# johncai117/Meta-Fine-Tuning

Hardware: AMD Instinct MI355X
Metric: episodes/sec at 5-way N-shot (ResNet10+GNN) per GPU and 1/2/4/8-GPU node (higher is better)
Workload: dtype f32

## Files before the change

### meta-fine-tuning_amd/csrc/conv_igemm.hip

```cpp
#include "mft_common.h"
#include "mft_hip_testing.h"

int mft_stem_conv_dispatch(const float* in, const float* w, float* out, int n_img, int H, int W, int w_ld,
                           hipStream_t s);
int mft_skinny_fwd_dispatch(const float* in, int ldi, const float* w, float* out, int ldo, int n_img, int H, int W,
                            int Cin, int Cout, int KH, int KW, int stride, int pad, int imgs_per_group,
                            long long w_group_stride, hipStream_t s);
void mft_skinny_set_dgrad_slices(int n);
void mft_skinny_set_tap(int v);
void mft_skinny_set_x3(int v);
void mft_skinny_set_nw(int v);
void mft_bn_small_set_rows(int rows);
void mft_bn_fwd_small_set_rows(int rows);
void mft_skinny_set_lines(int v);
int mft_skinny_dgrad_dispatch(const float* dy, int ldy, const float* w, float* dx, int ldx, int n_img, int H, int W,
                              int Cin, int Cout, int KH, int KW, int stride, int pad, int imgs_per_group,
                              long long w_group_stride, hipStream_t s);

namespace {

struct ConvArgs {
    const float* in;
    const float* w;
    const float* bias;
    float* out;
    int ldi, ldo;
    int H, W, Cin, OH, OW, Cout, KH, KW, stride, pad;
    int Kpad;
    int Ktot;
    int rows_per_group;
    int imgs_per_group;
    int tiles_n;
    long long wgs;
    int bt_stride;
    int ksplit;
    float* ws;
    int parity;
};

constexpr int BK = 32;
constexpr int LDS_LD = 36;
int g_dgrad_parity = 1;
int g_wgrad_tile = 64;
int g_conv_tile = 0;
int g_wgrad_pol = 7;
int g_wgrad_trim = 1;
int g_wgrad_rows = 1;
int g_wgrad_early = 1;
int g_wgrad_min_lds_kb = 0;
int g_skinny = 1;
int g_stem_fast = 1;

template <int BM, int BN, int WM, int WN, bool STEM, bool BT>
__global__ __launch_bounds__(256) void conv_igemm_kernel(ConvArgs p) {
    constexpr int TM = BM / WM / 32;
    constexpr int TN = BN / WN / 32;
    constexpr int PA = BM / 32;
    constexpr int PB = BN / 32;
    extern __shared__ __attribute__((aligned(16))) float smem[];

    const int tid = threadIdx.x;
    const int lane = tid & 63;
    const int wave = tid >> 6;
    const int wm = wave / WN, wn = wave % WN;
    const int r = lane & 31, h = lane >> 5;

    int tile_id = blockIdx.x;
    if (gridDim.y == 1) {
        const int nwg = gridDim.x, q = nwg >> 3, rmd = nwg & 7;
        const int xcd = tile_id & 7, slot = tile_id >> 3;
        tile_id = xcd * q + (xcd < rmd ? xcd : rmd) + slot;
    }
    const int nt = tile_id % p.tiles_n;
    const int mt = tile_id / p.tiles_n;
    const bool par = BT && p.parity != 0;
    const int g = par ? 0 : blockIdx.y;
    const int ph = par ? (int)(blockIdx.y >> 1) : 0, pw = par ? (int)(blockIdx.y & 1) : 0;
    const int Hc = par ? (p.OH - ph + 1) / 2 : p.OH, Wc = par ? (p.OW - pw + 1) / 2 : p.OW;
    const int rows = par ? p.imgs_per_group * Hc * Wc : p.rows_per_group;
    const int m0 = mt * BM, n0 = nt * BN;
    if (par && m0 >= rows) return;
    const int kh0 = par ? ((ph - p.pad) & 1) : 0, kw0 = par ? ((pw - p.pad) & 1) : 0;
    const int nkh = par ? (p.KH - kh0 + 1) / 2 : p.KH, nkw = par ? (p.KW - kw0 + 1) / 2 : p.KW;

    const int lrow = tid >> 3;
    const int c4 = (tid & 7) * 4;
    const int ohw = Hc * Wc;

    long long a_base[PA];
    int a_ih0[PA], a_iw0[PA];
    bool a_ok[PA];
// ... 1043 lines not shown
    a.Ktot = KH * KW * Cin;
    a.Kpad = (a.Ktot + 31) / 32 * 32;
    a.imgs_per_group = imgs_per_group;
    a.rows_per_group = imgs_per_group * a.OH * a.OW;
    a.wgs = (groups > 1) ? w_group_stride : 0;
    a.tiles_n = 0;
    a.bt_stride = 1;
    a.ksplit = 1; a.ws = nullptr; a.parity = 0;
    if (ws != nullptr && !stem && ldo % 4 == 0) {
        a.ksplit = conv_ksplit(a.rows_per_group, Cout, a.Kpad, groups);
        a.ws = ws;
    }
    hipStream_t s = (hipStream_t)stream;
    if (stem) {
        if (g_stem_fast && KH == 7 && KW == 7 && stride == 2 && pad == 3 && Cout == 64 && ldi == 3 && ldo == 64 &&
            bias == nullptr && (W == 84 || W == 224)) {
            const int rc = mft_stem_conv_dispatch(in, w, out, n_img, H, W, a.Kpad, s);
            if (rc != MFT_EINVAL) return rc;
        }
        return launch_conv<128, 64, 2, 2, true>(a, groups, s);
    }
    if (g_skinny && groups > 1 && w_group_stride != 0 && bias == nullptr && ws == nullptr) {
        const int rc = mft_skinny_fwd_dispatch(in, ldi, w, out, ldo, n_img, H, W, Cin, Cout, KH, KW, stride, pad,
                                               imgs_per_group, w_group_stride, s);
        if (rc != MFT_EINVAL) return rc;
    }
    int tile = g_conv_tile;
    if (tile == 0) tile = (Cout >= 64) ? 4 : 5;
    switch (tile) {
        case 1: return launch_conv<128, 128, 2, 2, false>(a, groups, s);
        case 2: return launch_conv<128, 64, 2, 2, false>(a, groups, s);
        case 3: return launch_conv<64, 128, 2, 2, false>(a, groups, s);
        case 4: return launch_conv<64, 64, 2, 2, false>(a, groups, s);
        default: return launch_conv<128, 32, 4, 1, false>(a, groups, s);
    }
}

extern "C" int mft_conv2d_nhwc(const float* in, int ldi, const float* w, const float* bias, float* out, int ldo,
                               int n_img, int H, int W, int Cin, int Cout, int KH, int KW, int stride, int pad,
                               int imgs_per_group, long long w_group_stride, void* stream) {
    return conv2d_impl(in, ldi, w, bias, out, ldo, n_img, H, W, Cin, Cout, KH, KW, stride, pad, imgs_per_group, w_group_stride,
                       nullptr, stream);
}

extern "C" long long mft_conv_ksplit_ws_floats(long long rows, int cols, int K) {
    const int s = conv_ksplit(rows, cols, K);
    return s > 1 ? (long long)s * rows * cols : 0;
}

extern "C" long long mft_conv_ksplit_grouped_ws_floats(long long rows_per_group, int cols, int K, int groups) {
    const int s = conv_ksplit(rows_per_group, cols, K, groups);
    return s > 1 ? (long long)s * groups * rows_per_group * cols : 0;
}

extern "C" int mft_conv2d_nhwc_ksplit_grouped(const float* in, int ldi, const float* w, float* out, int ldo, int n_img, int H, int W,
                                              int Cin, int Cout, int KH, int KW, int stride, int pad, int imgs_per_group,
                                              long long w_group_stride, float* ws, void* stream) {
    if (ws == nullptr || imgs_per_group <= 0) return MFT_EINVAL;
    return conv2d_impl(in, ldi, w, nullptr, out, ldo, n_img, H, W, Cin, Cout, KH, KW, stride, pad, imgs_per_group, w_group_stride, ws,
                       stream);
}

extern "C" int mft_conv2d_nhwc_ksplit(const float* in, int ldi, const float* w, const float* bias, float* out, int ldo,
                                      int n_img, int H, int W, int Cin, int Cout, int KH, int KW, int stride, int pad, float* ws,
                                      void* stream) {
    return conv2d_impl(in, ldi, w, bias, out, ldo, n_img, H, W, Cin, Cout, KH, KW, stride, pad, 0, 0, ws, stream);
}

extern "C" int mft_has_experiments(void) {
#ifdef MFT_EXPERIMENTS
    return 1;
#else
    return 0;
#endif
}

extern "C" int mft_debug_set_conv_tile(int tile) {
#ifndef MFT_EXPERIMENTS
    if (tile == 9502 || tile == 9504 || tile == 9505) return MFT_EINVAL;
    if (tile >= 9000 && tile < 9100 && tile != 9003 && tile != 9007) return MFT_EINVAL;
    if (tile > 4000 && tile < 5000) return MFT_EINVAL;
#endif
    if (tile >= 11000) { mft_bn_small_set_rows(tile - 11000); mft_bn_fwd_small_set_rows(tile - 11000); }
    else if (tile >= 9800) g_dgrad_parity = tile - 9800;
    else if (tile >= 9700) mft_skinny_set_lines(tile - 9700);
    else if (tile >= 9600) g_wgrad_trim = tile - 9600;
    else if (tile >= 9500) g_wgrad_rows = tile - 9500;
    else if (tile >= 9100) mft_skinny_set_nw(tile - 9100);
    else if (tile >= 9000) g_wgrad_pol = tile - 9000;
    else if (tile >= 8000) mft_skinny_set_x3(tile - 8000);
    else if (tile >= 7000) mft_skinny_set_tap(tile - 7000);
    else if (tile >= 6000) mft_skinny_set_dgrad_slices(tile - 6000);
    else if (tile >= 5000) g_wgrad_early = tile - 5000;
    else if (tile >= 4000) g_wgrad_min_lds_kb = tile - 4000;
    else if (tile >= 3000) g_skinny = tile - 3000;
    else if (tile >= 2100) g_stem_wgrad_strips = tile - 2100;
    else if (tile >= 2000) g_stem_fast = tile - 2000;
    else if (tile >= 1000) g_wgrad_tile = tile - 1000;
    else g_conv_tile = tile;
    return 0;
}

extern "C" int mft_debug_set_x3_tile(int t);

extern "C" void mft_wgrad_fwd_set_exact(int on);
extern "C" int mft_debug_reset(void) {
    mft_wgrad_fwd_set_exact(0);
    mft_wgrad_fwd_set_xcd(1);
    g_dgrad_parity = 1; g_wgrad_trim = 1; g_wgrad_rows = 1; g_wgrad_tile = 64; g_conv_tile = 0; g_wgrad_pol = 7; g_wgrad_early = 1; g_wgrad_min_lds_kb = 0; g_skinny = 1; g_stem_fast = 1; g_stem_wgrad_strips = 1;
    mft_skinny_set_lines(1); mft_skinny_set_nw(0); mft_skinny_set_x3(1); mft_skinny_set_tap(1); mft_skinny_set_dgrad_slices(1);
    mft_debug_set_x3_tile(0); mft_debug_set_x3_tile(10); mft_debug_set_x3_tile(21); mft_debug_set_x3_tile(31); mft_debug_set_x3_tile(41);
    mft_bn_small_set_rows(512); mft_bn_fwd_small_set_rows(512);
    mft_debug_set_x3_tile(60); mft_debug_set_x3_tile(70); mft_debug_set_x3_tile(80); mft_debug_set_x3_tile(91); mft_debug_set_x3_tile(100); mft_debug_set_x3_tile(200);
    return 0;
}

static int dgrad_impl(const float* dy, int ldy, const float* w, float* dx, int ldx, int n_img, int H,
                      int W, int Cin, int Cout, int KH, int KW, int stride, int pad,
                      int imgs_per_group, long long w_group_stride, float* ws, void* stream) {
    if (Cout % 32 != 0 || Cin % 4 != 0 || ldy % 4 != 0 || stride < 1) return MFT_EINVAL;
    if (imgs_per_group <= 0) imgs_per_group = n_img;
    if (n_img % imgs_per_group != 0) return MFT_EINVAL;
    const int groups = n_img / imgs_per_group;
    if (g_skinny && groups > 1 && w_group_stride != 0 && ws == nullptr) {
        const int rc = mft_skinny_dgrad_dispatch(dy, ldy, w, dx, ldx, n_img, H, W, Cin, Cout, KH, KW, stride, pad,
                                                 imgs_per_group, w_group_stride, (hipStream_t)stream);
        if (rc != MFT_EINVAL) return rc;
    }
    ConvArgs a;
    a.in = dy; a.w = w; a.bias = nullptr; a.out = dx;
    a.ldi = ldy; a.ldo = ldx;
    a.H = (H + 2 * pad - KH) / stride + 1;
    a.W = (W + 2 * pad - KW) / stride + 1;
    a.Cin = Cout; a.KH = KH; a.KW = KW;
    a.stride = 1; a.pad = -pad;
    a.bt_stride = stride;
    a.OH = H; a.OW = W;
    a.Cout = Cin;
    a.Ktot = KH * KW * Cout;
    a.Kpad = a.Ktot;
    a.imgs_per_group = imgs_per_group;
    a.rows_per_group = imgs_per_group * H * W;
    a.wgs = (groups > 1) ? w_group_stride : 0;
    a.tiles_n = 0;
    a.ksplit = 1; a.ws = nullptr;
    a.parity = (groups == 1 && stride == 2 && g_dgrad_parity) ? 1 : 0;
    if (ws != nullptr && ldx % 4 == 0 && Cin % 64 == 0) {
        const int s_full = conv_ksplit(a.rows_per_group, Cin, a.Kpad, groups);
        if (!a.parity) {
            a.ksplit = s_full;
            a.ws = ws;
        } else if (s_full > 1) {
            int sp = conv_ksplit((long long)imgs_per_group * ((H + 1) / 2) * ((W + 1) / 2), Cin, ((KH + 1) / 2) * ((KW + 1) / 2) * Cout, 4);
            if (sp > s_full) sp = s_full;
            if (sp > 1) { a.ksplit = sp; a.ws = ws; }
        }
    }
    hipStream_t s = (hipStream_t)stream;
    if (Cin % 64 == 0) return launch_conv<64, 64, 2, 2, false, true>(a, groups, s);
    return launch_conv<128, 32, 4, 1, false, true>(a, groups, s);
}

extern "C" int mft_conv2d_dgrad_nhwc(const float* dy, int ldy, const float* w, float* dx, int ldx, int n_img, int H,
                                     int W, int Cin, int Cout, int KH, int KW, int stride, int pad,
                                     int imgs_per_group, long long w_group_stride, void* stream) {
    return dgrad_impl(dy, ldy, w, dx, ldx, n_img, H, W, Cin, Cout, KH, KW, stride, pad, imgs_per_group, w_group_stride, nullptr,
                      stream);
}

extern "C" int mft_conv2d_dgrad_nhwc_ksplit_grouped(const float* dy, int ldy, const float* w, float* dx, int ldx, int n_img, int H,
                                                    int W, int Cin, int Cout, int KH, int KW, int stride, int pad, int imgs_per_group,
                                                    long long w_group_stride, float* ws, void* stream) {
    if (ws == nullptr || imgs_per_group <= 0 || stride != 1) return MFT_EINVAL;
    return dgrad_impl(dy, ldy, w, dx, ldx, n_img, H, W, Cin, Cout, KH, KW, stride, pad, imgs_per_group, w_group_stride, ws, stream);
}

extern "C" int mft_conv2d_dgrad_nhwc_ksplit(const float* dy, int ldy, const float* w, float* dx, int ldx, int n_img, int H, int W,
                                            int Cin, int Cout, int KH, int KW, int stride, int pad, float* ws, void* stream) {
    return dgrad_impl(dy, ldy, w, dx, ldx, n_img, H, W, Cin, Cout, KH, KW, stride, pad, 0, 0, ws, stream);
}

extern "C" long long mft_conv2d_wgrad_ws_floats(int n_img, int H, int W, int Cin, int Cout, int KH, int KW, int stride,
                                                 int pad, int imgs_per_group) {
    if (imgs_per_group <= 0) imgs_per_group = n_img;
    const int OH = (H + 2 * pad - KH) / stride + 1, OW = (W + 2 * pad - KW) / stride + 1;
    const long long rows = (long long)imgs_per_group * OH * OW;
    int chunk_rows, chunks;
    wgrad_chunking(rows, wgrad_wgs_per_chunk(Cin, Cout, KH, KW, n_img / imgs_per_group), &chunk_rows, &chunks);
    if (chunks <= 1) return 0;
    const long long kpad = (KH * KW * Cin + 31) / 32 * 32;
    return (long long)(n_img / imgs_per_group) * chunks * Cout * kpad;
}

// ... 122 lines not shown
```

### meta-fine-tuning_amd/csrc/skinny.hip

```cpp
#include "mft_common.h"

namespace {

typedef float f32x4v __attribute__((ext_vector_type(4)));

struct SkinnyArgs {
    const float* act;
    const float* w;
    float* out;
    int lda, ldo;
    int H, W, Cin, OH, OW, Cout, KH, KW, stride, pad;
    int ipg, rows_in, rows_out;
    long long wgs;
    int K;
    int CS;
};

constexpr int SK_PADF = 8;
constexpr int SK_U = 8;

__global__ __launch_bounds__(1024) void skinny_conv_fwd_kernel(SkinnyArgs p) {
    extern __shared__ __attribute__((aligned(16))) float lds[];
    const int tid = threadIdx.x;
    const int lane = tid & 63, wave = tid >> 6;
// ... 718 lines not shown
    auto wptr = [&](int qq) { return qq < n_groups ? sk_wptr<LN>(wrow, qq, p.K) : sk_wptr<LN>(wsrow, qq - n_groups, p.Cin); };
    f32x4v a_cur[SK_U];
#pragma unroll
    for (int u = 0; u < SK_U; ++u) a_cur[u] = __builtin_nontemporal_load((const f32x4v*)sk_wptr<LN>(wrow, u, p.K));
    gather(0);
    scatter(0);
    __syncthreads();
    auto pass_body = [&](int pass, f32x4v (&A)[3]) {
        const unsigned short* L = ldh + (pass & 1) * 3 * PL + 8 * kq;
        for (int cg0 = 0; cg0 < gpt; cg0 += SK_U) {
            const int q0 = pass * gpt + cg0;
            const bool more = q0 + SK_U < n_groups + gpt;
#pragma unroll
            for (int u = 0; u < SK_U; u += 2) {
                bf16x8 a[3], b[3][3];
                sk_wfix<LN>(a_cur[u], a_cur[u + 1]);
                sk_split_a(a_cur[u], a_cur[u + 1], a);
                if (more) {
                    a_cur[u] = __builtin_nontemporal_load((const f32x4v*)wptr(q0 + SK_U + u));
                    a_cur[u + 1] = __builtin_nontemporal_load((const f32x4v*)wptr(q0 + SK_U + u + 1));
                }
#pragma unroll
                for (int nb = 0; nb < 3; ++nb)
#pragma unroll
                    for (int pl = 0; pl < 3; ++pl)
                        b[nb][pl] = __builtin_bit_cast(bf16x8, *(const u32x4v*)(L + pl * PL + (nb * 16 + m) * RS + (cg0 + u) * 16));
                SK_X3_MFMA(A, a, b)
            }
        }
    };
    for (int pass = 0; pass < taps; ++pass) {
        gather(pass + 1);
        pass_body(pass, acc);
        scatter((pass + 1) & 1);
        __syncthreads();
    }
    pass_body(taps, acs);

    const float inv = 1.f / (float)p.rows_out;
    f32x4v s = {0.f, 0.f, 0.f, 0.f};
#pragma unroll
    for (int nb = 0; nb < 3; ++nb)
        if (nb * 16 + m < p.rows_out) s += acc[nb];
    f32x4v mu, rs;
#pragma unroll
    for (int e = 0; e < 4; ++e) mu[e] = sk_row16_sum(s[e]) * inv;
    s = f32x4v{0.f, 0.f, 0.f, 0.f};
#pragma unroll
    for (int nb = 0; nb < 3; ++nb)
        if (nb * 16 + m < p.rows_out) {
            const f32x4v d = acc[nb] - mu;
            s += d * d;
        }
#pragma unroll
    for (int e = 0; e < 4; ++e) rs[e] = 1.0f / sqrtf(sk_row16_sum(s[e]) * inv + q.eps);
    const int co = co0 + 4 * kq;
    const f32x4v ga = *(const f32x4v*)(q.gamma + g * q.gbs + co), be = *(const f32x4v*)(q.beta + g * q.gbs + co);
    if (m == 0) {
        *(f32x4v*)(q.mean + (long long)g * p.Cout + co) = mu;
        *(f32x4v*)(q.rstd + (long long)g * p.Cout + co) = rs;
    }
    const long long ob = (long long)g * p.rows_out * p.ldo;
#pragma unroll
    for (int nb = 0; nb < 3; ++nb) {
        const int ro = nb * 16 + m;
        if (ro >= p.rows_out) continue;
        const long long o = ob + (long long)ro * p.ldo + co;
        *(f32x4v*)(p.out + o) = acc[nb];
        *(f32x4v*)(q.sc + o) = acs[nb];
        f32x4v y = (acc[nb] - mu) * rs * ga + be;
#pragma unroll
        for (int e = 0; e < 4; ++e) y[e] = fmaxf(y[e], 0.f);
        *(f32x4v*)(q.r1 + o) = y;
    }
}

struct SkinnyBnArgs {
    const float* x_raw;
    const float* relu_out;
    const float* mean; const float* rstd; const float* gamma; long long gbs;
    float* dgamma; float* dbeta;
};

template <bool BNB, int NW>
__global__ __launch_bounds__(64 * NW) void skinny_conv_dgrad_x3_kernel(SkinnyArgs p, SkinnyBnArgs bn) {
    extern __shared__ __attribute__((aligned(16))) unsigned short ldh[];
    typedef float f32x2v __attribute__((ext_vector_type(2)));
    const int tid = threadIdx.x;
    const int lane = tid & 63, wave = tid >> 6;
    const int m = lane & 15, kq = lane >> 4;
    const int g = blockIdx.y;
    const int ci0 = blockIdx.x * (32 * NW) + wave * 32;
    const int Cdy = p.Cin, Cdx = p.Cout;
    const int RS = Cdy + SK_PADH;
    const int PL = p.rows_in * RS;
    const int hw = p.H * p.W;
    const int taps = p.KH * p.KW;
    const long long co_stride = (long long)taps * Cdx;

    int n_img[3], n_h[3], n_w[3];
    bool n_ok[3];
#pragma unroll
    for (int nb = 0; nb < 3; ++nb) {
        const int ro = nb * 16 + m;
        n_ok[nb] = ro < p.rows_out;
        const int rr = n_ok[nb] ? ro : 0;
        const int img = rr / hw;
        const int rem = rr - img * hw;
        n_img[nb] = img;
        n_h[nb] = rem / p.W;
        n_w[nb] = rem - n_h[nb] * p.W;
    }
    const float* wbase = p.w + (long long)g * p.wgs + ci0 + 2 * m;
    const float* actg = p.act + (long long)g * p.rows_in * p.lda;

    constexpr int U = 4;
    const int gpt = Cdy / 16;
    const int n_groups = taps * gpt;
    f32x2v a_cur[U][4];
    auto load_group = [&](int q, f32x2v* dst) {
        const int tap = q / gpt;
        const int cg = q - tap * gpt;
#pragma unroll
        for (int t = 0; t < 4; ++t) {
            const int co = cg * 16 + 4 * kq + t;
            dst[t] = __builtin_nontemporal_load((const f32x2v*)(wbase + (long long)co * co_stride + (long long)tap * Cdx));
        }
    };
#pragma unroll
    for (int u = 0; u < U; ++u) load_group(u, a_cur[u]);
    {
        const int q4 = Cdy / 4;
        for (int i = tid; i < p.rows_in * q4; i += 64 * NW) {
            const int r = i / q4, c = (i - r * q4) * 4;
            sk_store3(ldh, r * RS + sk_perm(c), PL, *(const f32x4v*)(actg + (long long)r * p.lda + c));
        }
    }
    __syncthreads();

    f32x4v acc[2][3];
#pragma unroll
    for (int b = 0; b < 2; ++b)
#pragma unroll
        for (int nb = 0; nb < 3; ++nb) acc[b][nb] = f32x4v{0.f, 0.f, 0.f, 0.f};

    for (int q0 = 0; q0 < n_groups; q0 += U) {
        const bool more = q0 + U < n_groups;
        const int tap = q0 / gpt;
        const int cg0 = q0 - tap * gpt;
        const int kh = tap / p.KW, kw = tap - kh * p.KW;
        int boff[3];
#pragma unroll
        for (int nb = 0; nb < 3; ++nb) {
            const int ih = n_h[nb] + p.pad - kh, iw = n_w[nb] + p.pad - kw;
            const bool ok = n_ok[nb] && ih >= 0 && ih < p.H && iw >= 0 && iw < p.W;
            boff[nb] = ok ? ((n_img[nb] * p.H + ih) * p.W + iw) * RS + 8 * kq + cg0 * 16 : -1;
        }
#pragma unroll
        for (int u = 0; u < U; u += 2) {
            bf16x8 a[2][3], b[3][3];
#pragma unroll
            for (int bb = 0; bb < 2; ++bb) {
                const f32x4v w0 = {a_cur[u][0][bb], a_cur[u][1][bb], a_cur[u][2][bb], a_cur[u][3][bb]};
                const f32x4v w1 = {a_cur[u + 1][0][bb], a_cur[u + 1][1][bb], a_cur[u + 1][2][bb], a_cur[u + 1][3][bb]};
                sk_split_a(w0, w1, a[bb]);
            }
            if (more) {
                load_group(q0 + U + u, a_cur[u]);
                load_group(q0 + U + u + 1, a_cur[u + 1]);
            }
#pragma unroll
            for (int nb = 0; nb < 3; ++nb)
#pragma unroll
                for (int pl = 0; pl < 3; ++pl) {
                    u32x4v z = {0u, 0u, 0u, 0u};
                    if (boff[nb] >= 0) z = *(const u32x4v*)(ldh + pl * PL + boff[nb] + u * 16);
                    b[nb][pl] = __builtin_bit_cast(bf16x8, z);
                }
            SK_X3_MFMA(acc[0], a[0], b)
            SK_X3_MFMA(acc[1], a[1], b)
        }
    }
    float* outg = p.out + (long long)g * p.rows_out * p.ldo;
    f32x4v d[3][2];
#pragma unroll
    for (int nb = 0; nb < 3; ++nb) {
        d[nb][0][0] = acc[0][nb][0]; d[nb][0][1] = acc[1][nb][0]; d[nb][0][2] = acc[0][nb][1]; d[nb][0][3] = acc[1][nb][1];
        d[nb][1][0] = acc[0][nb][2]; d[nb][1][1] = acc[1][nb][2]; d[nb][1][2] = acc[0][nb][3]; d[nb][1][3] = acc[1][nb][3];
    }
    const int cc = ci0 + 8 * kq;
    if constexpr (BNB) {
        const long long gb = (long long)g * p.rows_out * p.ldo;
        f32x4v mu[2], rs[2], ga[2], xh[3][2], s1[2], s2[2];
#pragma unroll
        for (int h = 0; h < 2; ++h) {
            mu[h] = *(const f32x4v*)(bn.mean + (long long)g * Cdx + cc + 4 * h);
            rs[h] = *(const f32x4v*)(bn.rstd + (long long)g * Cdx + cc + 4 * h);
            ga[h] = *(const f32x4v*)(bn.gamma + g * bn.gbs + cc + 4 * h);
            s1[h] = s2[h] = f32x4v{0.f, 0.f, 0.f, 0.f};
        }
#pragma unroll
        for (int nb = 0; nb < 3; ++nb) {
            const int ro = nb * 16 + m;
#pragma unroll
            for (int h = 0; h < 2; ++h) {
                xh[nb][h] = f32x4v{0.f, 0.f, 0.f, 0.f};
                if (ro < p.rows_out) {
                    const long long o = gb + (long long)ro * p.ldo + cc + 4 * h;
                    const f32x4v r = *(const f32x4v*)(bn.relu_out + o);
                    xh[nb][h] = (*(const f32x4v*)(bn.x_raw + o) - mu[h]) * rs[h];
#pragma unroll
                    for (int e = 0; e < 4; ++e) d[nb][h][e] = r[e] > 0.f ? d[nb][h][e] : 0.f;
                    s1[h] += d[nb][h];
                    s2[h] += d[nb][h] * xh[nb][h];
                } else {
                    d[nb][h] = f32x4v{0.f, 0.f, 0.f, 0.f};
                }
            }
        }
        const float inv = 1.f / (float)p.rows_out;
#pragma unroll
        for (int h = 0; h < 2; ++h) {
#pragma unroll
            for (int e = 0; e < 4; ++e) {
                s1[h][e] = sk_row16_sum(s1[h][e]);
                s2[h][e] = sk_row16_sum(s2[h][e]);
            }
            if (m == 0) {
                *(f32x4v*)(bn.dgamma + (long long)g * Cdx + cc + 4 * h) = s2[h];
                *(f32x4v*)(bn.dbeta + (long long)g * Cdx + cc + 4 * h) = s1[h];
            }
            const f32x4v m1 = s1[h] * inv, m2 = s2[h] * inv, kk = ga[h] * rs[h];
#pragma unroll
            for (int nb = 0; nb < 3; ++nb) d[nb][h] = kk * (d[nb][h] - m1 - xh[nb][h] * m2);
        }
    }
#pragma unroll
    for (int nb = 0; nb < 3; ++nb) {
        const int ro = nb * 16 + m;
        if (ro >= p.rows_out) continue;
        float* o = outg + (long long)ro * p.ldo + cc;
        *(f32x4v*)(o) = d[nb][0];
        *(f32x4v*)(o + 4) = d[nb][1];
    }
}

int g_skinny_x3 = 1;
int g_skinny_tap = 1;
int g_skinny_dgrad_slices = 1;

int g_skinny_lines = 1;
int g_skinny_nw = 0;

inline int pick_nw(int groups, int wgs_per_group_at_max, int nw_max) {
    if (g_skinny_nw == 0) return nw_max;
    if (g_skinny_nw != 99) return g_skinny_nw <= nw_max ? (g_skinny_nw >= nw_max / 4 ? g_skinny_nw : nw_max / 4) : nw_max;
    int nw = nw_max;
    while (nw > nw_max / 4 && (long long)groups * wgs_per_group_at_max * (nw_max / nw) < 256) nw >>= 1;
    return nw;
}

template <typename K, typename... A>
int launch_big_lds(K kern, size_t max_lds, dim3 grid, dim3 block, size_t lds, hipStream_t s, A... args) {
    static std::mutex mu;
    static const void* done[256];
    static int done_dev[256];
    static int n_done = 0;
    int dev = 0;
    (void)hipGetDevice(&dev);
    bool seen = false;
    {
        std::lock_guard<std::mutex> lock(mu);
        for (int i = 0; i < n_done; ++i) seen = seen || (done[i] == (const void*)kern && done_dev[i] == dev);
    }
    if (!seen) {
        hipError_t e = hipFuncSetAttribute((const void*)kern, hipFuncAttributeMaxDynamicSharedMemorySize, (int)max_lds);
        if (e != hipSuccess) return (int)e;
        std::lock_guard<std::mutex> lock(mu);
        bool dup = false;
        for (int i = 0; i < n_done; ++i) dup = dup || (done[i] == (const void*)kern && done_dev[i] == dev);
        if (!dup && n_done < 256) { done[n_done] = (const void*)kern; done_dev[n_done] = dev; ++n_done; }
    }
    hipLaunchKernelGGL(kern, grid, block, lds, s, args...);
    return mft_launch_status();
}

int pick_slice(int rows_in, int Cin) {
    for (int cs = Cin; cs >= 128; cs /= 2) {
        if (cs % 128 != 0 || Cin % cs != 0) continue;
        if ((long long)rows_in * (cs + SK_PADF) * 4 <= 100 * 1024) return cs;
    }
    return 0;
}

}

void mft_skinny_set_dgrad_slices(int n) { g_skinny_dgrad_slices = n; }
void mft_skinny_set_tap(int v) { g_skinny_tap = v; }
void mft_skinny_set_x3(int v) { g_skinny_x3 = v; }
void mft_skinny_set_nw(int v) { g_skinny_nw = v; }
void mft_skinny_set_lines(int v) { g_skinny_lines = v; }

static int skinny_fwd_impl(const float* in, int ldi, const float* w, float* out, int ldo, int n_img, int H, int W,
                           int Cin, int Cout, int KH, int KW, int stride, int pad, int imgs_per_group,
                           long long w_group_stride, const SkinnyExitArgs* ex, hipStream_t s) {
    if (imgs_per_group <= 0 || w_group_stride == 0 || n_img % imgs_per_group != 0) return MFT_EINVAL;
    const int OH = (H + 2 * pad - KH) / stride + 1, OW = (W + 2 * pad - KW) / stride + 1;
    const int rows_out = imgs_per_group * OH * OW, rows_in = imgs_per_group * H * W;
    if (rows_out > 48 || Cout % 256 != 0 || Cin % 128 != 0 || ldi % 4 != 0 || ldo % 4 != 0) return MFT_EINVAL;
    const int cs = pick_slice(rows_in, Cin);
    SkinnyArgs p;
    p.act = in; p.w = w; p.out = out; p.lda = ldi; p.ldo = ldo;
    p.H = H; p.W = W; p.Cin = Cin; p.OH = OH; p.OW = OW; p.Cout = Cout; p.KH = KH; p.KW = KW; p.stride = stride; p.pad = pad;
    p.ipg = imgs_per_group; p.rows_in = rows_in; p.rows_out = rows_out; p.wgs = w_group_stride;
    p.K = KH * KW * Cin; p.CS = cs;
    dim3 grid(Cout / 256, n_img / imgs_per_group, 1);
    if (cs != Cin) {
        if (ex != nullptr) return MFT_EINVAL;
        if (Cin > 256 || Cin % (16 * SK_U) != 0 || g_skinny_tap == 0) return MFT_EINVAL;
        if (g_skinny_x3) {
            const size_t lds_h = (size_t)2 * 3 * 48 * (Cin + SK_PADH) * 2;
            static bool attr_tx = false;
            if (!attr_tx) {
                hipError_t e = hipFuncSetAttribute((const void*)skinny_conv_fwd_tap_x3_kernel<true>,
                                                   hipFuncAttributeMaxDynamicSharedMemorySize, 156 * 1024);
                if (e == hipSuccess)
                    e = hipFuncSetAttribute((const void*)skinny_conv_fwd_tap_x3_kernel<false>,
                                            hipFuncAttributeMaxDynamicSharedMemorySize, 156 * 1024);
                if (e != hipSuccess) return (int)e;
                attr_tx = true;
            }
            if (g_skinny_lines) hipLaunchKernelGGL(skinny_conv_fwd_tap_x3_kernel<true>, grid, dim3(1024), lds_h, s, p);
            else hipLaunchKernelGGL(skinny_conv_fwd_tap_x3_kernel<false>, grid, dim3(1024), lds_h, s, p);
            return mft_launch_status();
        }
        const size_t lds_t = (size_t)2 * 48 * (Cin + SK_PADF) * sizeof(float);
        static bool attr_t = false;
        if (!attr_t) {
            hipError_t e = hipFuncSetAttribute((const void*)skinny_conv_fwd_tap_kernel,
                                               hipFuncAttributeMaxDynamicSharedMemorySize, 110 * 1024);
            if (e != hipSuccess) return (int)e;
            attr_t = true;
        }
        hipLaunchKernelGGL(skinny_conv_fwd_tap_kernel, grid, dim3(1024), lds_t, s, p);
        return mft_launch_status();
    }
    if (g_skinny_x3 && (size_t)3 * rows_in * (Cin + SK_PADH) * 2 <= 150 * 1024 && Cin % (16 * SK_U) == 0) {
        size_t lds3 = (size_t)3 * rows_in * (Cin + SK_PADH) * 2;
        if (ex != nullptr && lds3 < (size_t)16 * 48 * 16 * 4) lds3 = (size_t)16 * 48 * 16 * 4;
        const int groups = n_img / imgs_per_group;
        const int nw = pick_nw(groups, Cout / 256, 16);
        const dim3 g2(Cout / (16 * nw), groups, 1);
        const SkinnyExitArgs e0 = ex ? *ex : SkinnyExitArgs{};
#define SK_FWD(EX, NW) (g_skinny_lines ? launch_big_lds(skinny_conv_fwd_x3_kernel<EX, NW, true>, 150 * 1024, g2, dim3(64 * NW), lds3, s, p, e0) \
                                       : launch_big_lds(skinny_conv_fwd_x3_kernel<EX, NW, false>, 150 * 1024, g2, dim3(64 * NW), lds3, s, p, e0))
        if (ex != nullptr) return nw == 16 ? SK_FWD(true, 16) : nw == 8 ? SK_FWD(true, 8) : SK_FWD(true, 4);
        return nw == 16 ? SK_FWD(false, 16) : nw == 8 ? SK_FWD(false, 8) : SK_FWD(false, 4);
#undef SK_FWD
    }
    if (ex != nullptr) return MFT_EINVAL;
    const size_t lds = (size_t)rows_in * (cs + SK_PADF) * sizeof(float);
    static MftPerDeviceOnce attr_once;
    if (attr_once.need()) {
        hipError_t e = hipFuncSetAttribute((const void*)skinny_conv_fwd_kernel, hipFuncAttributeMaxDynamicSharedMemorySize,
                                           110 * 1024);
        if (e != hipSuccess) return (int)e;
        attr_once.mark();
    }
    hipLaunchKernelGGL(skinny_conv_fwd_kernel, grid, dim3(1024), lds, s, p);
    return mft_launch_status();
}

static int skinny_dgrad_impl(const float* dy, int ldy, const float* w, float* dx, int ldx, int n_img, int H, int W,
                             int Cin, int Cout, int KH, int KW, int stride, int pad, int imgs_per_group,
                             long long w_group_stride, const SkinnyBnArgs* bn, hipStream_t s) {
    if (imgs_per_group <= 0 || w_group_stride == 0 || n_img % imgs_per_group != 0 || stride != 1) return MFT_EINVAL;
    if (2 * pad != KH - 1 || 2 * pad != KW - 1) return MFT_EINVAL;
    const int rows = imgs_per_group * H * W;
    if (rows > 48 || Cin % 256 != 0 || Cout % 64 != 0 || ldy % 4 != 0 || ldx % 4 != 0) return MFT_EINVAL;
    int cs = Cout;
    if (g_skinny_dgrad_slices > 1 && Cout % (64 * g_skinny_dgrad_slices) == 0) cs = Cout / g_skinny_dgrad_slices;
    if ((long long)rows * (cs + SK_PADF) * 4 > 100 * 1024) return MFT_EINVAL;
    SkinnyArgs p;
    p.act = dy; p.w = w; p.out = dx; p.lda = ldy; p.ldo = ldx;
    p.H = H; p.W = W; p.Cin = Cout; p.OH = H; p.OW = W; p.Cout = Cin; p.KH = KH; p.KW = KW; p.stride = 1; p.pad = pad;
    p.ipg = imgs_per_group; p.rows_in = rows; p.rows_out = rows; p.wgs = w_group_stride;
    p.K = KH * KW * Cin; p.CS = cs;
    dim3 grid(Cin / 256, n_img / imgs_per_group, 1);
    if (g_skinny_x3 && g_skinny_dgrad_slices <= 1 && (size_t)3 * rows * (Cout + SK_PADH) * 2 <= 150 * 1024 && Cout % 64 == 0) {
        const size_t lds3 = (size_t)3 * rows * (Cout + SK_PADH) * 2;
        const int groups = n_img / imgs_per_group;
        int nw = pick_nw(groups, Cin / 256, 8);
        if (nw > 8) nw = 8;
        const dim3 g2(Cin / (32 * nw), groups, 1);
        const SkinnyBnArgs b0 = bn ? *bn : SkinnyBnArgs{};
#define SK_DG(BB, NW) launch_big_lds(skinny_conv_dgrad_x3_kernel<BB, NW>, 150 * 1024, g2, dim3(64 * NW), lds3, s, p, b0)
        if (bn != nullptr) return nw == 8 ? SK_DG(true, 8) : nw == 4 ? SK_DG(true, 4) : SK_DG(true, 2);
        return nw == 8 ? SK_DG(false, 8) : nw == 4 ? SK_DG(false, 4) : SK_DG(false, 2);
#undef SK_DG
    }
    if (bn != nullptr) return MFT_EINVAL;
    const size_t lds = (size_t)rows * (cs + SK_PADF) * sizeof(float);
    static MftPerDeviceOnce attr_once;
    if (attr_once.need()) {
        hipError_t e = hipFuncSetAttribute((const void*)skinny_conv_dgrad_kernel, hipFuncAttributeMaxDynamicSharedMemorySize,
                                           110 * 1024);
        if (e != hipSuccess) return (int)e;
        attr_once.mark();
    }
    hipLaunchKernelGGL(skinny_conv_dgrad_kernel, grid, dim3(512), lds, s, p);
    return mft_launch_status();
}

int mft_skinny_fwd_dispatch(const float* in, int ldi, const float* w, float* out, int ldo, int n_img, int H, int W,
                            int Cin, int Cout, int KH, int KW, int stride, int pad, int imgs_per_group,
                            long long w_group_stride, hipStream_t s) {
    return skinny_fwd_impl(in, ldi, w, out, ldo, n_img, H, W, Cin, Cout, KH, KW, stride, pad, imgs_per_group, w_group_stride,
                           nullptr, s);
}

extern "C" int mft_block_exit_small_forward(const float* r1, const float* w_c2, long long w_group_stride, const float* sc,
                                            float* c2, float* out, float* pooled, int n_img, int H, int W, int C,
                                            int imgs_per_group, const float* gamma2, const float* beta2, const float* gamma_sc,
                                            const float* beta_sc, long long gb_group_stride, float* mean2, float* rstd2,
                                            float* mean_sc, float* rstd_sc, float eps, void* stream) {
    if (!sc || !out || !pooled || imgs_per_group <= 0) return MFT_EINVAL;
    SkinnyExitArgs ex{sc, out, pooled, gamma2, beta2, gamma_sc, beta_sc, gb_group_stride, mean2, rstd2, mean_sc, rstd_sc, eps,
                      H * W};
    return skinny_fwd_impl(r1, C, w_c2, c2, C, n_img, H, W, C, C, 3, 3, 1, 1, imgs_per_group, w_group_stride, &ex,
                           (hipStream_t)stream);
}

int mft_skinny_dgrad_dispatch(const float* dy, int ldy, const float* w, float* dx, int ldx, int n_img, int H, int W,
                              int Cin, int Cout, int KH, int KW, int stride, int pad, int imgs_per_group,
                              long long w_group_stride, hipStream_t s) {
    return skinny_dgrad_impl(dy, ldy, w, dx, ldx, n_img, H, W, Cin, Cout, KH, KW, stride, pad, imgs_per_group, w_group_stride,
                             nullptr, s);
}

extern "C" int mft_conv2d_dgrad_bn_backward_small(const float* dy, int ldy, const float* w, float* dx, int ldx, int n_img, int H,
                                                  int W, int Cin, int Cout, int KH, int KW, int pad, int imgs_per_group,
                                                  long long w_group_stride, const float* x_raw, const float* relu_out,
                                                  const float* mean, const float* rstd, const float* gamma,
                                                  long long gb_group_stride, float* dgamma, float* dbeta, void* stream) {
    if (!x_raw || !relu_out || !mean || !rstd || !gamma || !dgamma || !dbeta || ldx != Cin) return MFT_EINVAL;
    SkinnyBnArgs bn{x_raw, relu_out, mean, rstd, gamma, gb_group_stride, dgamma, dbeta};
    return skinny_dgrad_impl(dy, ldy, w, dx, ldx, n_img, H, W, Cin, Cout, KH, KW, 1, pad, imgs_per_group, w_group_stride, &bn,
                             (hipStream_t)stream);
}

extern "C" int mft_block_entry_small_forward(const float* x, int ldx, const float* w_c1, long long w1_group_stride,
                                             const float* w_sc, long long wsc_group_stride, float* c1, float* r1, float* sc,
                                             int n_img, int H, int W, int Cin, int Cout, int stride, int imgs_per_group,
                                             const float* gamma1, const float* beta1, long long gb_group_stride, float* mean1,
                                             float* rstd1, float eps, void* stream) {
    if (imgs_per_group <= 0 || n_img % imgs_per_group != 0 || w1_group_stride == 0 || wsc_group_stride == 0) return MFT_EINVAL;
    const int OH = (H + 2 - 3) / stride + 1, OW = (W + 2 - 3) / stride + 1;
    if ((H - 1) / stride + 1 != OH || (W - 1) / stride + 1 != OW) return MFT_EINVAL;
    const int rows_out = imgs_per_group * OH * OW;
    if (!g_skinny_x3 || rows_out > 48 || Cout % 256 != 0 || Cin % (16 * SK_U) != 0 || Cin > 256 || ldx % 4 != 0) return MFT_EINVAL;
    SkinnyEntryArgs q;
    SkinnyArgs& p = q.c;
    p.act = x; p.w = w_c1; p.out = c1; p.lda = ldx; p.ldo = Cout;
    p.H = H; p.W = W; p.Cin = Cin; p.OH = OH; p.OW = OW; p.Cout = Cout; p.KH = 3; p.KW = 3; p.stride = stride; p.pad = 1;
    p.ipg = imgs_per_group; p.rows_in = imgs_per_group * H * W; p.rows_out = rows_out; p.wgs = w1_group_stride;
    p.K = 9 * Cin; p.CS = Cin;
    q.w_sc = w_sc; q.wscs = wsc_group_stride; q.sc = sc; q.r1 = r1; q.gamma = gamma1; q.beta = beta1; q.gbs = gb_group_stride;
    q.mean = mean1; q.rstd = rstd1; q.eps = eps;
    const size_t lds_h = (size_t)2 * 3 * 48 * (Cin + SK_PADH) * 2;
    const int groups = n_img / imgs_per_group;
    const int nw = pick_nw(groups, Cout / 256, 16);
    const dim3 g2(Cout / (16 * nw), groups, 1);
#define SK_EN(NW) (g_skinny_lines ? launch_big_lds(skinny_block_entry_x3_kernel<NW, true>, 156 * 1024, g2, dim3(64 * NW), lds_h, (hipStream_t)stream, q) \
                                  : launch_big_lds(skinny_block_entry_x3_kernel<NW, false>, 156 * 1024, g2, dim3(64 * NW), lds_h, (hipStream_t)stream, q))
    return nw == 16 ? SK_EN(16) : nw == 8 ? SK_EN(8) : SK_EN(4);
#undef SK_EN
}
```

Measured before the change: 90.29.

## Add sliced double-buffered LDS variant of skinny dgrad x3 kernel

Adds a new skinny dgrad kernel that stages the dy activations in 64-channel slices. Each slice is double-buffered in a small LDS footprint, with register prefetch of the next slice, instead of loading the whole channel range into up to 150KB of LDS. The aim is to cut LDS per block so more blocks or waves fit per CU (waves_per_eu 3) and to overlap global loads with MFMA work. It is used by default when nw==8. The shared epilogue is factored into a helper. The trade-off is a __syncthreads per slice and re-reading the LDS tile per tap.

```diff
diff --git a/meta-fine-tuning_amd/csrc/conv_igemm.hip b/meta-fine-tuning_amd/csrc/conv_igemm.hip
--- a/meta-fine-tuning_amd/csrc/conv_igemm.hip
+++ b/meta-fine-tuning_amd/csrc/conv_igemm.hip
@@ -7,6 +7,7 @@
                             int Cin, int Cout, int KH, int KW, int stride, int pad, int imgs_per_group,
                             long long w_group_stride, hipStream_t s);
 void mft_skinny_set_dgrad_slices(int n);
+void mft_skinny_set_dgrad_small(int v);
 void mft_skinny_set_tap(int v);
 void mft_skinny_set_x3(int v);
 void mft_skinny_set_nw(int v);
@@ -1216,6 +1217,7 @@
     if (tile > 4000 && tile < 5000) return MFT_EINVAL;
 #endif
     if (tile >= 11000) { mft_bn_small_set_rows(tile - 11000); mft_bn_fwd_small_set_rows(tile - 11000); }
+    else if (tile >= 9900) mft_skinny_set_dgrad_small(tile - 9900);
     else if (tile >= 9800) g_dgrad_parity = tile - 9800;
     else if (tile >= 9700) mft_skinny_set_lines(tile - 9700);
     else if (tile >= 9600) g_wgrad_trim = tile - 9600;
@@ -1242,7 +1244,7 @@
     mft_wgrad_fwd_set_exact(0);
     mft_wgrad_fwd_set_xcd(1);
     g_dgrad_parity = 1; g_wgrad_trim = 1; g_wgrad_rows = 1; g_wgrad_tile = 64; g_conv_tile = 0; g_wgrad_pol = 7; g_wgrad_early = 1; g_wgrad_min_lds_kb = 0; g_skinny = 1; g_stem_fast = 1; g_stem_wgrad_strips = 1;
-    mft_skinny_set_lines(1); mft_skinny_set_nw(0); mft_skinny_set_x3(1); mft_skinny_set_tap(1); mft_skinny_set_dgrad_slices(1);
+    mft_skinny_set_lines(1); mft_skinny_set_nw(0); mft_skinny_set_x3(1); mft_skinny_set_tap(1); mft_skinny_set_dgrad_slices(1); mft_skinny_set_dgrad_small(1);
     mft_debug_set_x3_tile(0); mft_debug_set_x3_tile(10); mft_debug_set_x3_tile(21); mft_debug_set_x3_tile(31); mft_debug_set_x3_tile(41);
     mft_bn_small_set_rows(512); mft_bn_fwd_small_set_rows(512);
     mft_debug_set_x3_tile(60); mft_debug_set_x3_tile(70); mft_debug_set_x3_tile(80); mft_debug_set_x3_tile(91); mft_debug_set_x3_tile(100); mft_debug_set_x3_tile(200);
diff --git a/meta-fine-tuning_amd/csrc/skinny.hip b/meta-fine-tuning_amd/csrc/skinny.hip
--- a/meta-fine-tuning_amd/csrc/skinny.hip
+++ b/meta-fine-tuning_amd/csrc/skinny.hip
@@ -824,6 +824,74 @@
     float* dgamma; float* dbeta;
 };
 
+template <bool BNB>
+__device__ __forceinline__ void sk_dgrad_epilogue(const f32x4v (&acc)[2][3], const SkinnyArgs& p, const SkinnyBnArgs& bn, int g,
+                                                  int ci0, int m, int kq) {
+    const int Cdx = p.Cout;
+    float* outg = p.out + (long long)g * p.rows_out * p.ldo;
+    f32x4v d[3][2];
+#pragma unroll
+    for (int nb = 0; nb < 3; ++nb) {
+        d[nb][0][0] = acc[0][nb][0]; d[nb][0][1] = acc[1][nb][0]; d[nb][0][2] = acc[0][nb][1]; d[nb][0][3] = acc[1][nb][1];
+        d[nb][1][0] = acc[0][nb][2]; d[nb][1][1] = acc[1][nb][2]; d[nb][1][2] = acc[0][nb][3]; d[nb][1][3] = acc[1][nb][3];
+    }
+    const int cc = ci0 + 8 * kq;
+    if constexpr (BNB) {
+        const long long gb = (long long)g * p.rows_out * p.ldo;
+        f32x4v mu[2], rs[2], ga[2], xh[3][2], s1[2], s2[2];
+#pragma unroll
+        for (int h = 0; h < 2; ++h) {
+            mu[h] = *(const f32x4v*)(bn.mean + (long long)g * Cdx + cc + 4 * h);
+            rs[h] = *(const f32x4v*)(bn.rstd + (long long)g * Cdx + cc + 4 * h);
+            ga[h] = *(const f32x4v*)(bn.gamma + g * bn.gbs + cc + 4 * h);
+            s1[h] = s2[h] = f32x4v{0.f, 0.f, 0.f, 0.f};
+        }
+#pragma unroll
+        for (int nb = 0; nb < 3; ++nb) {
+            const int ro = nb * 16 + m;
+#pragma unroll
+            for (int h = 0; h < 2; ++h) {
+                xh[nb][h] = f32x4v{0.f, 0.f, 0.f, 0.f};
+                if (ro < p.rows_out) {
+                    const long long o = gb + (long long)ro * p.ldo + cc + 4 * h;
+                    const f32x4v r = *(const f32x4v*)(bn.relu_out + o);
+                    xh[nb][h] = (*(const f32x4v*)(bn.x_raw + o) - mu[h]) * rs[h];
+#pragma unroll
+                    for (int e = 0; e < 4; ++e) d[nb][h][e] = r[e] > 0.f ? d[nb][h][e] : 0.f;
+                    s1[h] += d[nb][h];
+                    s2[h] += d[nb][h] * xh[nb][h];
+                } else {
+                    d[nb][h] = f32x4v{0.f, 0.f, 0.f, 0.f};
+                }
+            }
+        }
+        const float inv = 1.f / (float)p.rows_out;
+#pragma unroll
+        for (int h = 0; h < 2; ++h) {
+#pragma unroll
+            for (int e = 0; e < 4; ++e) {
+                s1[h][e] = sk_row16_sum(s1[h][e]);
+                s2[h][e] = sk_row16_sum(s2[h][e]);
+            }
+            if (m == 0) {
+                *(f32x4v*)(bn.dgamma + (long long)g * Cdx + cc + 4 * h) = s2[h];
+                *(f32x4v*)(bn.dbeta + (long long)g * Cdx + cc + 4 * h) = s1[h];
+            }
+            const f32x4v m1 = s1[h] * inv, m2 = s2[h] * inv, kk = ga[h] * rs[h];
+#pragma unroll
+            for (int nb = 0; nb < 3; ++nb) d[nb][h] = kk * (d[nb][h] - m1 - xh[nb][h] * m2);
+        }
+    }
+#pragma unroll
+    for (int nb = 0; nb < 3; ++nb) {
+        const int ro = nb * 16 + m;
+        if (ro >= p.rows_out) continue;
+        float* o = outg + (long long)ro * p.ldo + cc;
+        *(f32x4v*)(o) = d[nb][0];
+        *(f32x4v*)(o + 4) = d[nb][1];
+    }
+}
+
 template <bool BNB, int NW>
 __global__ __launch_bounds__(64 * NW) void skinny_conv_dgrad_x3_kernel(SkinnyArgs p, SkinnyBnArgs bn) {
     extern __shared__ __attribute__((aligned(16))) unsigned short ldh[];
@@ -923,73 +991,144 @@
             SK_X3_MFMA(acc[1], a[1], b)
         }
     }
-    float* outg = p.out + (long long)g * p.rows_out * p.ldo;
-    f32x4v d[3][2];
-#pragma unroll
-    for (int nb = 0; nb < 3; ++nb) {
-        d[nb][0][0] = acc[0][nb][0]; d[nb][0][1] = acc[1][nb][0]; d[nb][0][2] = acc[0][nb][1]; d[nb][0][3] = acc[1][nb][1];
-        d[nb][1][0] = acc[0][nb][2]; d[nb][1][1] = acc[1][nb][2]; d[nb][1][2] = acc[0][nb][3]; d[nb][1][3] = acc[1][nb][3];
-    }
-    const int cc = ci0 + 8 * kq;
-    if constexpr (BNB) {
-        const long long gb = (long long)g * p.rows_out * p.ldo;
-        f32x4v mu[2], rs[2], ga[2], xh[3][2], s1[2], s2[2];
-#pragma unroll
-        for (int h = 0; h < 2; ++h) {
-            mu[h] = *(const f32x4v*)(bn.mean + (long long)g * Cdx + cc + 4 * h);
-            rs[h] = *(const f32x4v*)(bn.rstd + (long long)g * Cdx + cc + 4 * h);
-            ga[h] = *(const f32x4v*)(bn.gamma + g * bn.gbs + cc + 4 * h);
-            s1[h] = s2[h] = f32x4v{0.f, 0.f, 0.f, 0.f};
-        }
-#pragma unroll
-        for (int nb = 0; nb < 3; ++nb) {
-            const int ro = nb * 16 + m;
-#pragma unroll
-            for (int h = 0; h < 2; ++h) {
-                xh[nb][h] = f32x4v{0.f, 0.f, 0.f, 0.f};
-                if (ro < p.rows_out) {
-                    const long long o = gb + (long long)ro * p.ldo + cc + 4 * h;
-                    const f32x4v r = *(const f32x4v*)(bn.relu_out + o);
-                    xh[nb][h] = (*(const f32x4v*)(bn.x_raw + o) - mu[h]) * rs[h];
-#pragma unroll
-                    for (int e = 0; e < 4; ++e) d[nb][h][e] = r[e] > 0.f ? d[nb][h][e] : 0.f;
-                    s1[h] += d[nb][h];
-                    s2[h] += d[nb][h] * xh[nb][h];
-                } else {
-                    d[nb][h] = f32x4v{0.f, 0.f, 0.f, 0.f};
-                }
-            }
-        }
-        const float inv = 1.f / (float)p.rows_out;
-#pragma unroll
-        for (int h = 0; h < 2; ++h) {
-#pragma unroll
-            for (int e = 0; e < 4; ++e) {
-                s1[h][e] = sk_row16_sum(s1[h][e]);
-                s2[h][e] = sk_row16_sum(s2[h][e]);
-            }
-            if (m == 0) {
-                *(f32x4v*)(bn.dgamma + (long long)g * Cdx + cc + 4 * h) = s2[h];
-                *(f32x4v*)(bn.dbeta + (long long)g * Cdx + cc + 4 * h) = s1[h];
-            }
-            const f32x4v m1 = s1[h] * inv, m2 = s2[h] * inv, kk = ga[h] * rs[h];
-#pragma unroll
-            for (int nb = 0; nb < 3; ++nb) d[nb][h] = kk * (d[nb][h] - m1 - xh[nb][h] * m2);
-        }
-    }
+    sk_dgrad_epilogue<BNB>(acc, p, bn, g, ci0, m, kq);
+}
+
+constexpr int SK_DSL = 64;
+constexpr int SK_DRS = SK_DSL + SK_PADH;
+
+template <bool BNB, int NW>
+__global__ __launch_bounds__(64 * NW) __attribute__((amdgpu_waves_per_eu(3))) void skinny_conv_dgrad_x3s_kernel(SkinnyArgs p, SkinnyBnArgs bn) {
+    extern __shared__ __attribute__((aligned(16))) unsigned short ldh[];
+    typedef float f32x2v __attribute__((ext_vector_type(2)));
+    const int tid = threadIdx.x;
+    const int lane = tid & 63, wave = tid >> 6;
+    const int m = lane & 15, kq = lane >> 4;
+    const int g = blockIdx.y;
+    const int ci0 = blockIdx.x * (32 * NW) + wave * 32;
+    const int Cdy = p.Cin, Cdx = p.Cout;
+    const int PL = p.rows_in * SK_DRS;
+    const int hw = p.H * p.W;
+    const int taps = p.KH * p.KW;
+    const long long co_stride = (long long)taps * Cdx;
+
+    int n_img[3], n_h[3], n_w[3];
+    bool n_ok[3];
 #pragma unroll
     for (int nb = 0; nb < 3; ++nb) {
         const int ro = nb * 16 + m;
-        if (ro >= p.rows_out) continue;
-        float* o = outg + (long long)ro * p.ldo + cc;
-        *(f32x4v*)(o) = d[nb][0];
-        *(f32x4v*)(o + 4) = d[nb][1];
-    }
-}
-
+        n_ok[nb] = ro < p.rows_out;
+        const int rr = n_ok[nb] ? ro : 0;
+        const int img = rr / hw;
+        const int rem = rr - img * hw;
+        n_img[nb] = img;
+        n_h[nb] = rem / p.W;
+        n_w[nb] = rem - n_h[nb] * p.W;
+    }
+    const float* wbase = p.w + (long long)g * p.wgs + ci0 + 2 * m;
+    const float* actg = p.act + (long long)g * p.rows_in * p.lda;
+
+    constexpr int U = SK_DSL / 16;
+    const int gpt = Cdy / 16;
+    const int spt = Cdy / SK_DSL;
+    const int n_groups = taps * gpt;
+    f32x2v a_cur[U][4];
+    auto load_group = [&](int q, f32x2v* dst) {
+        const int tap = q / gpt;
+        const int cg = q - tap * gpt;
+#pragma unroll
+        for (int t = 0; t < 4; ++t) {
+            const int co = cg * 16 + 4 * kq + t;
+            dst[t] = __builtin_nontemporal_load((const f32x2v*)(wbase + (long long)co * co_stride + (long long)tap * Cdx));
+        }
+    };
+#pragma unroll
+    for (int u = 0; u < U; ++u) load_group(u, a_cur[u]);
+
+    constexpr int NST = (48 * (SK_DSL / 4) + 64 * NW - 1) / (64 * NW);
+    const int n_st = p.rows_in * (SK_DSL / 4);
+    f32x4v st[NST];
+    auto stage_load = [&](int it) {
+        const float* src = actg + (it % spt) * SK_DSL;
+#pragma unroll
+        for (int j = 0; j < NST; ++j) {
+            const int i = tid + j * 64 * NW;
+            if (i < n_st) st[j] = *(const f32x4v*)(src + (long long)(i >> 4) * p.lda + (i & 15) * 4);
+        }
+    };
+    auto stage_store = [&](int buf) {
+        unsigned short* L = ldh + buf * 3 * PL;
+#pragma unroll
+        for (int j = 0; j < NST; ++j) {
+            const int i = tid + j * 64 * NW;
+            if (i < n_st) sk_store3(L, (i >> 4) * SK_DRS + sk_perm((i & 15) * 4), PL, st[j]);
+        }
+    };
+    const int n_it = n_groups / U;
+    stage_load(0);
+    stage_store(0);
+    if (n_it > 1) stage_load(1);
+    __syncthreads();
+
+    f32x4v acc[2][3];
+#pragma unroll
+    for (int b = 0; b < 2; ++b)
+#pragma unroll
+        for (int nb = 0; nb < 3; ++nb) acc[b][nb] = f32x4v{0.f, 0.f, 0.f, 0.f};
+
+    for (int it = 0; it < n_it; ++it) {
+        const int q0 = it * U;
+        const bool more = it + 1 < n_it;
+        if (more) stage_store((it + 1) & 1);
+        if (it + 2 < n_it) stage_load(it + 2);
+        const unsigned short* L = ldh + (it & 1) * 3 * PL;
+        const int tap = q0 / gpt;
+        const int kh = tap / p.KW, kw = tap - kh * p.KW;
+        int boff[3];
+#pragma unroll
+        for (int nb = 0; nb < 3; ++nb) {
+            const int ih = n_h[nb] + p.pad - kh, iw = n_w[nb] + p.pad - kw;
+            const bool ok = n_ok[nb] && ih >= 0 && ih < p.H && iw >= 0 && iw < p.W;
+            boff[nb] = ok ? ((n_img[nb] * p.H + ih) * p.W + iw) * SK_DRS + 8 * kq : -1;
+        }
+#pragma unroll
+        for (int u = 0; u < U; u += 2) {
+            bf16x8 a[2][3];
+#pragma unroll
+            for (int bb = 0; bb < 2; ++bb) {
+                const f32x4v w0 = {a_cur[u][0][bb], a_cur[u][1][bb], a_cur[u][2][bb], a_cur[u][3][bb]};
+                const f32x4v w1 = {a_cur[u + 1][0][bb], a_cur[u + 1][1][bb], a_cur[u + 1][2][bb], a_cur[u + 1][3][bb]};
+                sk_split_a(w0, w1, a[bb]);
+            }
+            if (more) {
+                load_group(q0 + U + u, a_cur[u]);
+                load_group(q0 + U + u + 1, a_cur[u + 1]);
+            }
+            constexpr int TA[6] = {2, 0, 1, 1, 0, 0}, TB[6] = {0, 2, 1, 0, 1, 0};
+#pragma unroll
+            for (int nb = 0; nb < 3; ++nb) {
+                bf16x8 b[3];
+#pragma unroll
+                for (int pl = 0; pl < 3; ++pl) {
+                    u32x4v z = {0u, 0u, 0u, 0u};
+                    if (boff[nb] >= 0) z = *(const u32x4v*)(L + pl * PL + boff[nb] + u * 16);
+                    b[pl] = __builtin_bit_cast(bf16x8, z);
+                }
+#pragma unroll
+                for (int t = 0; t < 6; ++t)
+#pragma unroll
+                    for (int bb = 0; bb < 2; ++bb)
+                        acc[bb][nb] = __builtin_amdgcn_mfma_f32_16x16x32_bf16(a[bb][TA[t]], b[TB[t]], acc[bb][nb], 0, 0, 0);
+            }
+        }
+        __syncthreads();
+    }
+    sk_dgrad_epilogue<BNB>(acc, p, bn, g, ci0, m, kq);
+}
 int g_skinny_x3 = 1;
 int g_skinny_tap = 1;
 int g_skinny_dgrad_slices = 1;
+int g_skinny_dgrad_small = 1;
 
 int g_skinny_lines = 1;
 int g_skinny_nw = 0;
@@ -1038,6 +1177,7 @@
 }
 
 void mft_skinny_set_dgrad_slices(int n) { g_skinny_dgrad_slices = n; }
+void mft_skinny_set_dgrad_small(int v) { g_skinny_dgrad_small = v; }
 void mft_skinny_set_tap(int v) { g_skinny_tap = v; }
 void mft_skinny_set_x3(int v) { g_skinny_x3 = v; }
 void mft_skinny_set_nw(int v) { g_skinny_nw = v; }
@@ -1136,6 +1276,12 @@
         if (nw > 8) nw = 8;
         const dim3 g2(Cin / (32 * nw), groups, 1);
         const SkinnyBnArgs b0 = bn ? *bn : SkinnyBnArgs{};
+        if (g_skinny_dgrad_small && nw == 8) {
+            const size_t lds_s = (size_t)2 * 3 * rows * SK_DRS * 2;
+            if (bn != nullptr) hipLaunchKernelGGL((skinny_conv_dgrad_x3s_kernel<true, 8>), g2, dim3(512), lds_s, s, p, b0);
+            else hipLaunchKernelGGL((skinny_conv_dgrad_x3s_kernel<false, 8>), g2, dim3(512), lds_s, s, p, b0);
+            return mft_launch_status();
+        }
 #define SK_DG(BB, NW) launch_big_lds(skinny_conv_dgrad_x3_kernel<BB, NW>, 150 * 1024, g2, dim3(64 * NW), lds3, s, p, b0)
         if (bn != nullptr) return nw == 8 ? SK_DG(true, 8) : nw == 4 ? SK_DG(true, 4) : SK_DG(true, 2);
         return nw == 8 ? SK_DG(false, 8) : nw == 4 ? SK_DG(false, 4) : SK_DG(false, 2);
```

New measurement: 90.17. Within noise of the previous version (-0.1%).
